# magenta/ddsp

Hardware: AMD Instinct MI355X
Metric: Msamples/s (Harmonic+FilteredNoise, 16kHz, 100 harmonics) (higher is better)
Workload: dtype f32 (Harmonic wavetables and the FilteredNoise FIR/IR products: 22-bit operands - fp16 hi/lo pairs on the MFMA matrix cores - with fp32 accumulation; everything else plain fp32, the frame phase prefix fp64)

## Files before the change

ddsp_amd/csrc/harmonic_table.hip:

```cpp
#include <hip/hip_runtime.h>
#include <hip/hip_ext.h>
#include <stdint.h>
#include <cstdlib>
#include <type_traits>
#include "../../include/ddsp_amd.h"
#include "common.h"
#include "split_f16.h"
#include "profile.h"
#include "harmonic_table.h"
#include "wavetable_coeffs.h"
#include "harm_table_frags.h"
#include "launch.h"
#include <mutex>

namespace ddsp {

static __device__ WtFragSet kWtFragSet6;
static __device__ WtFragSet kWtFragSet8;
static __device__ WtFragsWide kWtFragsWide;

constexpr int kWtT = 512;
constexpr int kWtHalf = kWtT / 2;
constexpr int kWtNQ = kWtT / 4;
template <int W> struct WtGeom {
  static constexpr int H = W <= 8 ? 4 : 8;
  static constexpr int TS = kWtHalf + 2 * H + 4;
};
constexpr int kWtRowTiles = 2;
constexpr int kWtRows = 16 * kWtRowTiles;
constexpr int kWtFrames = kWtRows - 1;
constexpr int kWtNT = 4;
template <int NK> struct WtPlane { static constexpr int PS = NK <= 2 ? 72 : 104; };

struct ChunkTables {
  double theta[kWtRows], w[kWtRows], dw[kWtRows];
  float f0[kWtRows + 2];
  int kA[kWtRows], kN[kWtRows];
  int cross;
  float4 cx[kWtRows];
  float ck[kWtRows];
};

template <int W> struct WtPoly;
template <> struct WtPoly<6> {
  static constexpr int DE = kWtDegE6, DO = kWtDegO6, K512 = 100;
  static constexpr float e(int p, int d) { return kWtE6[p * (DE + 1) + d]; }
  static constexpr float o(int p, int d) { return kWtO6[p * (DO + 1) + d]; }
};
template <> struct WtPoly<8> {
  static constexpr int DE = kWtDegE8, DO = kWtDegO8, K512 = 128;
  static constexpr float e(int p, int d) { return kWtE8[p * (DE + 1) + d]; }
  static constexpr float o(int p, int d) { return kWtO8[p * (DO + 1) + d]; }
};

template <> struct WtPoly<10> {
  static constexpr int DE = kWtDegE10, DO = kWtDegO10, K512 = 200;
  static constexpr float e(int p, int d) { return kWtE10[p * (DE + 1) + d]; }
  static constexpr float o(int p, int d) { return kWtO10[p * (DO + 1) + d]; }
};

constexpr int kWtWalker = 2;
constexpr int kWtSizer = 0;
constexpr unsigned kWtSlots = 0x73256104u;
struct WtDesc { int b, j0, nfr, fresh; };

struct WtSizeThresholds { float t64, t128, t256; };

struct TableArgs {
  int B, F, K, N, hop;
  int total_frames, frames_per_block;
  FastDiv f_div, tpf_div, seg_div;
  float nyquist, nyq_lo, nyq_hi;
  WtSizeThresholds size_thr;
  int amp_linear;
  int ragged;
  int rows16;
  double inv_sr, inv_2hop, hop_d, half_hm1;
};

struct WtWalk { int pos, pos_first, end, seg_left, base, rem, b, j; };

constexpr int kWtSegment = 2 * kWtFrames;

__device__ __forceinline__ WtDesc wt_next_chunk(WtWalk& w, const TableArgs& p) {
  WtDesc d{0, 0, 0, 0};
  if (w.pos >= w.end) return d;
  if (w.seg_left == 0) {
    uint32_t j;
    const int b = (int)fastdiv((uint32_t)w.pos, p.f_div, j);
    d.fresh = (w.pos == w.pos_first || (int)j == 0) ? 1 : 0;
    w.b = b;
    w.j = (int)j;
    uint32_t in_seg;
    (void)fastdiv(j, p.seg_div, in_seg);
    w.seg_left = min(min(w.end - w.pos, p.F - w.j), kWtSegment - (int)in_seg);
    const int n = (w.seg_left + kWtFrames - 1) / kWtFrames;
    w.base = w.seg_left / n;
    w.rem = w.seg_left - w.base * n;
  }
  const int len = w.base + (w.rem > 0 ? 1 : 0);
  if (w.rem > 0) --w.rem;
  d.b = w.b; d.j0 = w.j; d.nfr = len;
  w.pos += len; w.j += len; w.seg_left -= len;
  return d;
}

__device__ __forceinline__ int wt_table_size(float f0_min, const WtSizeThresholds& th) {
  return f0_min >= th.t64 ? 64 : f0_min >= th.t128 ? 128 : f0_min >= th.t256 ? 256 : kWtT;
}
inline WtSizeThresholds wt_size_thresholds(int K512, int K, float nyq_hi) {
  auto thr = [&](int T) -> float {
    const int kmax = K512 * T / 512;
    if (K <= kmax) return -__builtin_inff();
    return (float)((double)nyq_hi / (double)(kmax + 1) * (1.0 + 1e-6));
  };
  return WtSizeThresholds{thr(64), thr(128), thr(256)};
}

__device__ __forceinline__ WtDesc wt_read_desc(const WtDesc* ring, int slot) {
  const int4 v = *reinterpret_cast<const int4*>(ring + slot);
  WtDesc d;
  d.b = __builtin_amdgcn_readfirstlane(v.x);
  d.j0 = __builtin_amdgcn_readfirstlane(v.y);
  d.nfr = __builtin_amdgcn_readfirstlane(v.z);
  d.fresh = __builtin_amdgcn_readfirstlane(v.w);
  return d;
// ... 17 lines not shown
  __asm__("v_fma_mixhi_f16 %0, %1, %2, %3 op_sel:[1,0,0] op_sel_hi:[1,0,0]" : "+v"(r) : "v"(h), "v"(m), "v"(c2048[1]));
  return r;
#else
  return (h16x2){(__fp16)fmaf((float)h[0], -kLoScale, c2048[0]), (__fp16)fmaf((float)h[1], -kLoScale, c2048[1])};
#endif
}
__device__ __forceinline__ int wt_floor_int(float x) {
#if defined(__AMDGCN__)
  int r;
  __asm__("v_cvt_flr_i32_f32 %0, %1" : "=v"(r) : "v"(x));
  return r;
#else
  return (int)floorf(x);
#endif
}
__device__ __forceinline__ f32x2 wt_pk_fma_swap(f32x2 a, f32x2 b, f32x2 c) {
  return (f32x2){fmaf(a[0], b[1], c[0]), fmaf(a[1], b[0], c[1])};
}
__device__ __forceinline__ f32x2 wt_pk_plus(f32x2 o, f32x2 zz, f32x2 e) {
  return (f32x2){fmaf(o[0], zz[0], e[0]), fmaf(o[1], zz[0], e[1])};
}
__device__ __forceinline__ f32x2 wt_pk_minus(f32x2 o, f32x2 zz, f32x2 e) {
  return (f32x2){fmaf(-o[0], zz[0], e[0]), fmaf(-o[1], zz[0], e[1])};
}
template <int N>
__device__ __forceinline__ void wt_frags_landed(f32x4& a, f32x4& b, f32x4& c, f32x4& d) {
#if defined(__AMDGCN__)
  __asm__ volatile("s_waitcnt vmcnt(%4)" : "+v"(a), "+v"(b), "+v"(c), "+v"(d) : "n"(N));
#else
  (void)a; (void)b; (void)c; (void)d;
#endif
}
template <int N, class Fn>
__device__ __forceinline__ void wt_static_for(Fn&& f) {
  if constexpr (N > 0) {
    wt_static_for<N - 1>(f);
    f(std::integral_constant<int, N - 1>{});
  }
}
template <int W> struct WtPkCoefs {
  static constexpr int NG = W / 4, MID = (W / 2) & 1, DE = WtPoly<W>::DE, DO = WtPoly<W>::DO;
  f32x2 e[NG][DE + 1], o[NG][DO + 1], m[DE + 1];
  __device__ __forceinline__ void init() {
    wt_static_for<NG>([&](auto gg) {
      constexpr int g = decltype(gg)::value, pb = 2 * g + MID, pa = pb + 1;
      wt_static_for<DE + 1>([&](auto ss) {
// ... 66 lines not shown
    }
#pragma unroll
    for (int u = 0; u < NT; ++u) wp[u] = wt_pk_plus(oo[u], zz[u], ee[u]);
#pragma unroll
    for (int u = 0; u < NT; ++u) wm[u] = wt_pk_minus(oo[u], zz[u], ee[u]);
#pragma unroll
    for (int u = 0; u < NT; ++u) acc0[u] = wt_pk_fma(wp[u], lo0[u], acc0[u]);
#pragma unroll
    for (int u = 0; u < NT; ++u) acc1[u] = wt_pk_fma(wp[u], lo1[u], acc1[u]);
#pragma unroll
    for (int u = 0; u < NT; ++u) acc0[u] = wt_pk_fma_swap(wm[u], hi0[u], acc0[u]);
#pragma unroll
    for (int u = 0; u < NT; ++u) acc1[u] = wt_pk_fma_swap(wm[u], hi1[u], acc1[u]);
  });
}

typedef float* __restrict__ WtOutRestrict;
template <bool ADD> struct WtOut { typedef WtOutRestrict type; };
template <> struct WtOut<true> { typedef float* type; };

template <int W, int NK, bool ONE_TILE, bool ADD, bool ROWS16>
__global__ __launch_bounds__(1024) void harm_table_kernel(
    const float* __restrict__ amplitudes, const float* __restrict__ hd, const float* __restrict__ f0_all,
    typename WtOut<ADD>::type audio, float* __restrict__ ctl_amp, float* __restrict__ ctl_hd, const float* add_in, TableArgs p) {
  constexpr int kWtH = WtGeom<W>::H, kWtTS = WtGeom<W>::TS, kWtPS = WtPlane<NK>::PS;
  constexpr bool WIDE = NK > 2;
  __shared__ __attribute__((aligned(16))) float tab_all[2][kWtRows * kWtTS];
  __shared__ __attribute__((aligned(16))) _Float16 planes_all[3][4 * kWtRows * kWtPS];
  __shared__ ChunkTables t_all[2];
  __shared__ __attribute__((aligned(16))) WtDesc ring[8];
  __shared__ float amp_tab[3][kWtRows + 4];
  __shared__ int tsel[4];

  const int tid = threadIdx.x, lane = tid & 63;
  const int wave = __builtin_amdgcn_readfirstlane(tid >> 6);
  const bool is_t = wave < 4;
  const int F = p.F, K = p.K;
  const int K4 = (K + 3) >> 2;
  const float kLog10 = 2.302585092994046f;
  const int sub = lane >> 5, kq = lane & 31;
  const bool live = kq < K4;
  const float4* __restrict__ hd4 = reinterpret_cast<const float4*>(hd);
  const int mi = lane & 15, mg = lane >> 4;

  WtWalk walk;
  walk.pos = (int)blockIdx.x * p.frames_per_block;
  walk.pos_first = walk.pos;
  walk.end = min(walk.pos + p.frames_per_block, p.total_frames);
  walk.seg_left = 0; walk.base = 0; walk.rem = 0; walk.b = 0; walk.j = 0;
  if (wave == kWtWalker) {
    const WtDesc d0 = wt_next_chunk(walk, p), d1 = wt_next_chunk(walk, p);
    if (lane == 0) { ring[0] = d0; ring[1] = d1; }
  }
  __syncthreads();
  WtDesc dL{0, 0, 0, 0}, dA = wt_read_desc(ring, 0), dM{0, 0, 0, 0}, dB{0, 0, 0, 0};
  int pa = 0, pm = 2, pb = 1;

  int4 dnext = make_int4(0, 0, 0, 0);
  auto desc_issue = [&](int slot) { dnext = *reinterpret_cast<const int4*>(ring + slot); };
  auto desc_take = [&]() {
    dL.b = __builtin_amdgcn_readfirstlane(dnext.x);
    dL.j0 = __builtin_amdgcn_readfirstlane(dnext.y);
    dL.nfr = __builtin_amdgcn_readfirstlane(dnext.z);
    dL.fresh = __builtin_amdgcn_readfirstlane(dnext.w);
  };

  if (is_t) {
    const int rw = wave;
    f16x8 ahi[2][2][WIDE ? 1 : NK], alo[2][2][WIDE ? 1 : NK];
    int frag_T = 0;
    auto fetch_fragments = [&](int T) {
      const WtFragSet& set = W == 6 ? kWtFragSet6 : kWtFragSet8;
// ... 65 lines not shown
    auto fetch_segment = [&](const WtDesc& d, float& dst) {
      int lane_ = lane;
      DDSP_KEEP_IN_VGPR(lane_);
      uint32_t in_seg;
      (void)fastdiv((uint32_t)d.j0, p.seg_div, in_seg);
      load_issue(dst, f0_all + (size_t)d.b * F + min(d.j0 - (int)in_seg + lane_, F - 1));
    };
    auto fragments_landed = [&]() {
#if defined(__AMDGCN__)
      __asm__ volatile("s_waitcnt vmcnt(0)");
#pragma unroll
      for (int par = 0; par < 2; ++par)
#pragma unroll
        for (int tt = 0; tt < 2; ++tt)
#pragma unroll
          for (int ks = 0; ks < (WIDE ? 1 : NK); ++ks)
            __asm__ volatile("" : "+v"(ahi[par][tt][ks]), "+v"(alo[par][tt][ks]));
#endif
    };
    if constexpr (!WIDE) { fetch_fragments(kWtT); frag_T = kWtT; }
    int Tm = kWtT, Tm_ahead = kWtT;
    for (int tick = -2;; ++tick) {
      if (rw == 3 && dM.nfr > 0) {
        if (dM.fresh) before = row_prefix(dM);
        fetch_f0(dM);
      }
      WtDesc dN{0, 0, 0, 0};
      if (rw == 1 && dA.nfr > 0) fetch_amp(dA);
      if constexpr (!WIDE) {
        if (rw == kWtSizer) {
          dN = wt_read_desc(ring, (tick + 3) & 7);
          if (dN.nfr > 0) fetch_segment(dN, pseg);
          if (tick == -2 && dA.nfr > 0) fetch_segment(dA, pf_first);
        }
      }
      if constexpr (!WIDE) {
        Tm_ahead = tsel[(tick + 2) & 3];
        if (tick == -1) Tm = __builtin_amdgcn_readfirstlane(tsel[0]);
        if (dM.nfr > 0 && Tm != frag_T) {
          fetch_fragments(Tm);
          frag_T = Tm;
          fragments_landed();
        }
      }
      if (dM.nfr > 0 && !WIDE && Tm != kWtT) {
        if (rw < (Tm >> 6)) {
          const int half = Tm >> 1;
#pragma unroll
          for (int rt = 0; rt < kWtRowTiles; ++rt) {
            const _Float16* bsrc = planes_all[pm] + (16 * rt + mi) * kWtPS + 8 * mg;
            const float am = amp_tab[pm][16 * rt + mi], am_lo = am * (1.0f / kLoScale);
            f32x4 soe[2];
#pragma unroll
            for (int par = 0; par < 2; ++par) {
              const f16x8 bhi = *reinterpret_cast<const f16x8*>(bsrc + (0 * 2 + par) * kWtRows * kWtPS);
              const f16x8 blo = *reinterpret_cast<const f16x8*>(bsrc + (1 * 2 + par) * kWtRows * kWtPS);
              const f32x4 zero = {0.f, 0.f, 0.f, 0.f};
              const f32x4 acc = __builtin_amdgcn_mfma_f32_16x16x32_f16(ahi[par][0][0], bhi, zero, 0, 0, 0);
              f32x4 accx = __builtin_amdgcn_mfma_f32_16x16x32_f16(ahi[par][0][0], blo, zero, 0, 0, 0);
              accx = __builtin_amdgcn_mfma_f32_16x16x32_f16(alo[par][0][0], bhi, accx, 0, 0, 0);
              soe[par] = acc * am + accx * am_lo;
            }
            float* trow = tab_all[(tick + 1) & 1] + (16 * rt + mi) * kWtTS + kWtH;
            const int n0 = 16 * rw + 4 * mg;
            const f32x4 sp = soe[0] + soe[1], sm = soe[0] - soe[1];
            *reinterpret_cast<f32x4*>(trow + n0) = sp;
            *reinterpret_cast<f32x4*>(trow + (half - 4 - n0)) = (f32x4){sm.w, sm.z, sm.y, sm.x};
            if (n0 == 0) {
              *reinterpret_cast<f32x4*>(trow - 4) = (f32x4){-sp.w, -sp.z, -sp.y, -sp.x};
              *reinterpret_cast<f32x4*>(trow + half) = (f32x4){-sm.x, -sm.y, -sm.z, -sm.w};
            }
          }
        }
      } else if (dM.nfr > 0) {
#pragma unroll
       for (int rt = 0; rt < kWtRowTiles; ++rt) {
        const _Float16* bsrc = planes_all[pm] + (16 * rt + mi) * kWtPS + 8 * mg;
        f32x4 soe[2][2];
        const float am = amp_tab[pm][16 * rt + mi], am_lo = am * (1.0f / kLoScale);
#pragma unroll
        for (int par = 0; par < 2; ++par) {
          f32x4 acc[2], accx[2];
#pragma unroll
          for (int tt = 0; tt < 2; ++tt) {
            acc[tt] = (f32x4){0.f, 0.f, 0.f, 0.f};
            accx[tt] = (f32x4){0.f, 0.f, 0.f, 0.f};
          }
          if constexpr (WIDE) {
            f32x4 fr[NK][2][2];
            const char* fbase = reinterpret_cast<const char*>(kWtFragsWide.v) + 16384 * (rw * 2 + par);
            unsigned lane16 = 16u * (unsigned)lane;
            DDSP_KEEP_IN_VGPR(lane16);
            wt_static_for<NK>([&](auto kk) {
              constexpr int ks = decltype(kk)::value;
#pragma unroll
              for (int tt = 0; tt < 2; ++tt)
#pragma unroll
                for (int hl = 0; hl < 2; ++hl)
                  load_issue_spaced<1024 * ks>(fr[ks][tt][hl], fbase, lane16 + 4096u * (unsigned)(2 * tt + hl));
            });
            wt_static_for<NK>([&](auto kk) {
              constexpr int ks = decltype(kk)::value;
              const f16x8 bhi = *reinterpret_cast<const f16x8*>(bsrc + (0 * 2 + par) * kWtRows * kWtPS + wt_wide_kstep_base(ks));
              const f16x8 blo = *reinterpret_cast<const f16x8*>(bsrc + (1 * 2 + par) * kWtRows * kWtPS + wt_wide_kstep_base(ks));
              wt_frags_landed<4 * (NK - 1 - ks)>(fr[ks][0][0], fr[ks][0][1], fr[ks][1][0], fr[ks][1][1]);
#pragma unroll
              for (int tt = 0; tt < 2; ++tt)
                acc[tt] = __builtin_amdgcn_mfma_f32_16x16x32_f16(__builtin_bit_cast(f16x8, fr[ks][tt][0]), bhi, acc[tt], 0, 0, 0);
#pragma unroll
              for (int tt = 0; tt < 2; ++tt)
                accx[tt] = __builtin_amdgcn_mfma_f32_16x16x32_f16(__builtin_bit_cast(f16x8, fr[ks][tt][0]), blo, accx[tt], 0, 0, 0);
#pragma unroll
              for (int tt = 0; tt < 2; ++tt)
                accx[tt] = __builtin_amdgcn_mfma_f32_16x16x32_f16(__builtin_bit_cast(f16x8, fr[ks][tt][1]), bhi, accx[tt], 0, 0, 0);
            });
          } else {
#pragma unroll
          for (int ks = 0; ks < NK; ++ks) {
            const f16x8 bhi = *reinterpret_cast<const f16x8*>(bsrc + (0 * 2 + par) * kWtRows * kWtPS + 32 * ks);
            const f16x8 blo = *reinterpret_cast<const f16x8*>(bsrc + (1 * 2 + par) * kWtRows * kWtPS + 32 * ks);
#pragma unroll
            for (int tt = 0; tt < 2; ++tt)
              acc[tt] = __builtin_amdgcn_mfma_f32_16x16x32_f16(ahi[par][tt][ks], bhi, acc[tt], 0, 0, 0);
#pragma unroll
            for (int tt = 0; tt < 2; ++tt)
              accx[tt] = __builtin_amdgcn_mfma_f32_16x16x32_f16(ahi[par][tt][ks], blo, accx[tt], 0, 0, 0);
#pragma unroll
            for (int tt = 0; tt < 2; ++tt)
              accx[tt] = __builtin_amdgcn_mfma_f32_16x16x32_f16(alo[par][tt][ks], bhi, accx[tt], 0, 0, 0);
          }
          }
#pragma unroll
          for (int tt = 0; tt < 2; ++tt) soe[par][tt] = acc[tt] * am + accx[tt] * am_lo;
        }
        float* trow = tab_all[(tick + 1) & 1] + (16 * rt + mi) * kWtTS + kWtH;
#pragma unroll
        for (int tt = 0; tt < 2; ++tt) {
          const int n0 = 16 * (2 * rw + tt) + 4 * mg;
          const f32x4 so = soe[0][tt], se = soe[1][tt];
          const f32x4 sp = so + se;
          const f32x4 sm = so - se;
          *reinterpret_cast<f32x4*>(trow + n0) = sp;
          *reinterpret_cast<f32x4*>(trow + (kWtHalf - 4 - n0)) = (f32x4){sm.w, sm.z, sm.y, sm.x};
          if constexpr (kWtH == 4) {
          if (n0 == 0) {
            *reinterpret_cast<f32x4*>(trow - kWtH) = (f32x4){-sp.w, -sp.z, -sp.y, -sp.x};
            *reinterpret_cast<f32x4*>(trow + kWtHalf) = (f32x4){-sm.x, -sm.y, -sm.z, -sm.w};
          }
          } else {
          if (n0 < kWtH) {
            *reinterpret_cast<f32x4*>(trow - 4 - n0) = (f32x4){-sp.w, -sp.z, -sp.y, -sp.x};
            *reinterpret_cast<f32x4*>(trow + kWtHalf + n0) = (f32x4){-sm.x, -sm.y, -sm.z, -sm.w};
          }
          }
        }
       }
      }
      desc_issue((tick + 3) & 7);
// ... 20 lines not shown
          const unsigned hi15 = (unsigned)__builtin_amdgcn_readlane((int)(unsigned)((unsigned long long)bits15 >> 32), 15);
          const double first16 = __builtin_bit_cast(double, (long long)(((unsigned long long)hi15 << 32) | lo15));
          if (lane >= 16) incl += first16;
          const double s_excl = before + (incl - mine);
          const double run = p.hop_d * s_excl + (fa - (double)pf_first) * p.half_hm1;
          const double cyc = run * p.inv_sr;
          const float fmx = fmaxf(fj, fj1), fmn = fminf(fj, fj1);
          int kA = Kc, kN = Kc;
          if (fmx > 0.0f) kA = (int)fminf((float)Kc, floorf(p.nyq_lo * __builtin_amdgcn_rcpf(fmx)));
          if (fmn > 0.0f) kN = (int)fminf((float)Kc, floorf(p.nyq_hi * __builtin_amdgcn_rcpf(fmn)));
          kA = max(min(kA, kN), 0);
          const bool crossing = lane < nfr && kA < kN;
          const unsigned long long any = __builtin_amdgcn_ballot_w64(crossing);
          if (lane == 0) t.cross = any != 0ull ? 1 : 0;
          if (lane <= kWtRows) t.f0[lane] = fj;
          if (lane < kWtRows) {
            t.theta[lane] = cyc - floor(cyc);
            t.w[lane] = fa * p.inv_sr;
            t.dw[lane] = (fb - fa) * p.inv_sr * p.inv_2hop;
            t.kA[lane] = kA;
            t.kN[lane] = kN;
          }
          if (any != 0ull) {
            float4 cx = make_float4(0.0f, 0.0f, 0.0f, 0.0f);
            float ck = 0.0f;
            if (crossing) {
              const int k = kA;
              const float kfl = (float)(k + 1);
              const _Float16* pl = planes_all[pm] + ((k & 1) * kWtRows + lane) * kWtPS + (k >> 1);
              const float c0 = fmaf((float)pl[2 * kWtRows * kWtPS], 1.0f / kLoScale, (float)pl[0]);
              const float c1 = fmaf((float)pl[2 * kWtRows * kWtPS + kWtPS], 1.0f / kLoScale, (float)pl[kWtPS]);
              const float top = rn_mul(fj, kfl), bot = rn_mul(fj1, kfl);
              cx = make_float4(rn_mul(c0, amp_tab[pm][lane]), rn_mul(c1, amp_tab[pm][lane + 1]), top, rn_sub(bot, top));
              ck = kfl;
            }
            if (lane < kWtRows) { t.cx[lane] = cx; t.ck[lane] = ck; }
          }
          const long long bits31 = __builtin_bit_cast(long long, incl);
          const unsigned lo31 = (unsigned)__builtin_amdgcn_readlane((int)(unsigned)(bits31 & 0xffffffffll), 31);
          const unsigned hi31 = (unsigned)__builtin_amdgcn_readlane((int)(unsigned)((unsigned long long)bits31 >> 32), 31);
          before += __builtin_bit_cast(double, (long long)(((unsigned long long)hi31 << 32) | lo31));
        }
      }
      if (rw == 1 && dA.nfr > 0) {
        loads_landed(pamp);
        int lane_ = lane;
        DDSP_KEEP_IN_VGPR(lane_);
        const float a = exp_sigmoid_fast(pamp, kLog10, 2.0f, 1e-7f);
        if (lane_ <= kWtRows) amp_tab[pa][lane_] = a;
        if (ctl_amp != nullptr && lane_ < dA.nfr) ctl_amp[(size_t)dA.b * F + dA.j0 + lane_] = a;
      }
      if (rw == kWtSizer && (dN.nfr > 0 || (tick == -2 && dA.nfr > 0))) {
        loads_landed(pseg, pf_first);
        int lane_ = lane;
// ... 31 lines not shown
      const int hq = WIDE ? lane : kq;
      const bool live_h = WIDE ? lane < K4 : live;
      auto row_of = [&](int i, int pass) -> int { return 2 * u0 + NU * pass + i; };
      float kf[4], nyq_u[4];
#pragma unroll
      for (int u = 0; u < 4; ++u) {
        const bool alive = 4 * hq + u + 1 <= K;
        kf[u] = alive ? (float)(4 * hq + u + 1) : 0.0f;
        nyq_u[u] = alive ? p.nyquist : -1.0f;
      }
      struct Rows { f32x4 x[NU]; float f0[NU]; };
      Rows rows_a, rows_b;
      const unsigned kq16 = 16u * (unsigned)min(hq, K4 - 1), row_bytes = 4u * (unsigned)K;
      unsigned ku4[4];
#pragma unroll
      for (int u = 0; u < 4; ++u) ku4[u] = 4u * (unsigned)min(4 * hq + u, K - 1);
      auto prefetch = [&](const WtDesc& d, Rows& r, int pass) {
        const size_t r0 = (size_t)d.b * (size_t)F;
        const char* hb = reinterpret_cast<const char*>(hd) + r0 * row_bytes;
        const char* fb = reinterpret_cast<const char*>(f0_all) + r0 * 4;
        unsigned ro[NU];
#pragma unroll
        for (int i = 0; i < NU; ++i) {
          const unsigned jr = (unsigned)min(WIDE ? d.j0 + row_of(i, pass) : d.j0 + 2 * (u0 + i) + sub, F - 1);
          ro[i] = __umul24(jr, row_bytes);
          if constexpr (WIDE) load_issue_spaced<0>(r.f0[i], fb, 4u * jr);
          else load_issue(r.f0[i], fb, 4u * jr);
        }
        if constexpr (ROWS16) {
#pragma unroll
          for (int i = 0; i < NU; ++i) {
            if constexpr (WIDE) load_issue_spaced<0>(r.x[i], hb, ro[i] + kq16);
            else load_issue(r.x[i], hb, ro[i] + kq16);
          }
        } else {
#pragma unroll
          for (int i = 0; i < NU; ++i) {
            float e0, e1, e2, e3;
            if constexpr (WIDE) {
              load_issue_spaced<0>(e0, hb, ro[i] + ku4[0]);
              load_issue_spaced<0>(e1, hb, ro[i] + ku4[1]);
              load_issue_spaced<0>(e2, hb, ro[i] + ku4[2]);
              load_issue_spaced<0>(e3, hb, ro[i] + ku4[3]);
            } else {
            load_issue(e0, hb, ro[i] + ku4[0]);
            load_issue(e1, hb, ro[i] + ku4[1]);
            load_issue(e2, hb, ro[i] + ku4[2]);
// ... 8 lines not shown
        __asm__ volatile("s_waitcnt vmcnt(0)" : "+v"(r.x[0]), "+v"(r.x[1]), "+v"(r.x[2]), "+v"(r.x[3]), "+v"(r.f0[0]), "+v"(r.f0[1]),
                         "+v"(r.f0[2]), "+v"(r.f0[3]));
#else
        (void)r;
#endif
      };
      const f32x2 kf_o = {kf[0], kf[2]}, kf_e = {kf[1], kf[3]};
      auto exp_sigmoid2 = [&](f32x2 v) -> f32x2 {
        const f32x2 t = v * -1.4426950408889634f;
        const f32x2 e = (f32x2){__builtin_amdgcn_exp2f(t[0]), __builtin_amdgcn_exp2f(t[1])} + 1.0f;
        const f32x2 m = (f32x2){__builtin_amdgcn_logf(e[0]), __builtin_amdgcn_logf(e[1])} * -kLog10;
        const f32x2 g = {__builtin_amdgcn_exp2f(m[0]), __builtin_amdgcn_exp2f(m[1])};
        return __builtin_elementwise_fma(g, (f32x2){2.0f, 2.0f}, (f32x2){1e-7f, 1e-7f});
      };
      const float kHuge = 0x1p100f;
      const f32x2 nyq_o = {nyq_u[0] * kHuge, nyq_u[2] * kHuge}, nyq_e = {nyq_u[1] * kHuge, nyq_u[3] * kHuge};
      auto nyq_mask2 = [&](f32x2 e, float f0r, f32x2 kfp, f32x2 nyq_s) -> f32x2 {
        f32x2 prod;
        { _Pragma("clang fp contract(off)") prod = kfp * f0r; }
        const f32x2 y = __builtin_elementwise_fma(prod, (f32x2){-kHuge, -kHuge}, nyq_s);
        return (f32x2){__builtin_amdgcn_fmed3f(e[0], 0.0f, y[0]), __builtin_amdgcn_fmed3f(e[1], 0.0f, y[1])};
      };
      auto phase_a = [&](const WtDesc& d, _Float16* planes, const Rows& r, int pass) {
        const int nfr = d.nfr;
        f32x2 xo[NU], xe[NU];
        float part[NU], inv[NU];
#pragma unroll
        for (int i = 0; i < NU; ++i) {
          xo[i] = nyq_mask2(exp_sigmoid2((f32x2){r.x[i][0], r.x[i][2]}), r.f0[i], kf_o, nyq_o);
          xe[i] = nyq_mask2(exp_sigmoid2((f32x2){r.x[i][1], r.x[i][3]}), r.f0[i], kf_e, nyq_e);
        }
#pragma unroll
        for (int i = 0; i < NU; ++i) { const f32x2 h = xo[i] + xe[i]; part[i] = h[0] + h[1]; }
#pragma unroll
        for (int i = 0; i < NU; ++i) part[i] += dpp_mov0<0xB1, 0xF>(part[i]);
#pragma unroll
        for (int i = 0; i < NU; ++i) part[i] += dpp_mov0<0x4E, 0xF>(part[i]);
#pragma unroll
        for (int i = 0; i < NU; ++i) part[i] += dpp_mov0<0x141, 0xF>(part[i]);
#pragma unroll
        for (int i = 0; i < NU; ++i) part[i] += dpp_mov0<0x140, 0xF>(part[i]);
#pragma unroll
        for (int i = 0; i < NU; ++i) {
          part[i] = row_pair_sum(part[i]);
          if constexpr (WIDE) part[i] = wave_half_sum(part[i]);
          inv[i] = __builtin_amdgcn_rcpf(fmaxf(part[i], 1e-7f));
        }
        if (ctl_hd != nullptr) {
#pragma unroll
          for (int i = 0; i < NU; ++i) {
            const int arow = WIDE ? row_of(i, pass) : 2 * (u0 + i) + sub;
            const int crow = d.b * F + d.j0 + arow;
            if (arow < nfr) {
              const f32x2 ho = xo[i] * inv[i], he = xe[i] * inv[i];
              if constexpr (ROWS16) {
                if (live_h) reinterpret_cast<float4*>(ctl_hd)[(size_t)crow * K4 + hq] = make_float4(ho[0], he[0], ho[1], he[1]);
              } else {
                float* __restrict__ crow_p = ctl_hd + (size_t)crow * K + 4 * hq;
                const float h4[4] = {ho[0], he[0], ho[1], he[1]};
#pragma unroll
                for (int u = 0; u < 4; ++u)
                  if (4 * hq + u < K) crow_p[u] = h4[u];
              }
            }
          }
        }
#pragma unroll
        for (int i = 0; i < NU; ++i) {
          const f32x2 c[2] = {xo[i] * inv[i], xe[i] * inv[i]};
          _Float16* dst = planes + (WIDE ? row_of(i, pass) : 2 * (u0 + i) + sub) * kWtPS + 2 * hq;
#pragma unroll
          for (int par = 0; par < 2; ++par) {
            const h16x2 hi = __builtin_amdgcn_cvt_pkrtz(c[par][0], c[par][1]);
            const h16x2 lo = wt_rest_halves(c[par] * kLoScale, hi);
            if (!WIDE || 2 * hq < kWtPS) {
              *reinterpret_cast<h16x2*>(dst + (0 * 2 + par) * kWtRows * kWtPS) = hi;
              *reinterpret_cast<h16x2*>(dst + (1 * 2 + par) * kWtRows * kWtPS) = lo;
            }
          }
        }
      };
      prefetch(dA, rows_a, 0);
      if constexpr (WIDE) prefetch(dA, rows_b, 1);
      auto one_tick = [&](int tick, Rows& cur, Rows& next) -> bool {
        desc_issue((tick + 3) & 7);
        desc_take();
        rows_landed(cur);
        if constexpr (WIDE) {
          rows_landed(next);
          if (dA.nfr > 0) phase_a(dA, planes_all[pa], cur, 0);
          prefetch(dL, cur, 0);
          if (dA.nfr > 0) phase_a(dA, planes_all[pa], next, 1);
          prefetch(dL, next, 1);
        } else {
        prefetch(dL, next, 0);
        if (dA.nfr > 0) phase_a(dA, planes_all[pa], cur, 0);
        }
        __syncthreads();
        dB = dM; dM = dA; dA = dL;
        { const int t3 = pb; pb = pm; pm = pa; pa = t3; }
// ... 93 lines not shown
              out[u] = __builtin_bit_cast(float, __builtin_bit_cast(unsigned, v) ^ sgn[u]);
            }
            if (chunk_cross)
#pragma unroll
            for (int u = 0; u < NT; ++u) {
              const int kA = __builtin_amdgcn_readfirstlane(t.kA[q[u]]);
              const int kN = __builtin_amdgcn_readfirstlane(t.kN[q[u]]);
              if (kA < kN) {
                {
                  const float4 cx = t.cx[q[u]];
                  const float ck = t.ck[q[u]];
                  const float fk = rn_add(cx.z, rn_mul(cx.w, lerp[u]));
                  const float ak = fmaf(w_next[u], cx.y, rn_mul(w_cur[u], cx.x));
                  const float sv = sin_rev(fmaf(theta[u], ck, -rintf(theta[u] * ck)));
                  if (fk >= p.nyquist) out[u] = fmaf(-ak, sv, out[u]);
                }
                if (kA + 1 < kN) {
                  const float fj = t.f0[q[u]], fj1 = t.f0[q[u] + 1];
                  const float am0 = amp_tab[pb][q[u]], am1 = amp_tab[pb][q[u] + 1];
                  for (int k = kA + 1; k < kN; ++k) {
                    const float kfl = (float)(k + 1);
                    const float top = fj * kfl, bot = fj1 * kfl;
                    const float fk = rn_add(top, rn_mul(rn_sub(bot, top), lerp[u]));
                    const _Float16* pl = planes + ((k & 1) * kWtRows + q[u]) * kWtPS + (k >> 1);
                    const float c0 = fmaf((float)pl[2 * kWtRows * kWtPS], 1.0f / kLoScale, (float)pl[0]);
                    const float c1 = fmaf((float)pl[2 * kWtRows * kWtPS + kWtPS], 1.0f / kLoScale, (float)pl[kWtPS]);
                    const float ak = fmaf(w_next[u], rn_mul(c1, am1), rn_mul(w_cur[u], rn_mul(c0, am0)));
                    const float sv = sin_rev(fmaf(theta[u], kfl, -rintf(theta[u] * kfl)));
                    if (fk >= p.nyquist) out[u] = fmaf(-ak, sv, out[u]);
                  }
                }
              }
            }
            if (ADD)
#pragma unroll
              for (int u = 0; u < NT; ++u) out[u] += addv[u];
            if (!ragged) {
#pragma unroll
              for (int u = 0; u < NT; ++u) *reinterpret_cast<float*>(out_chunk + (o32 + 2048u * (unsigned)u)) = out[u];
            } else {
#pragma unroll
              for (int u = 0; u < NT; ++u)
                if (r[u] < hop) *reinterpret_cast<float*>(out_chunk + 4u * (unsigned)(q[u] * hop + r[u])) = out[u];
            }
          };
          for (int base = 0; base < n_tiles; base += kWtFrames) {
            const int left = min(n_tiles - base, kWtFrames);
            const int cnt = (left - slot + 7) >> 3;
            if (cnt >= 4) tiles(base + slot, std::integral_constant<int, 4>{});
            else if (cnt == 3) tiles(base + slot, std::integral_constant<int, 3>{});
            else if (cnt == 2) tiles(base + slot, std::integral_constant<int, 2>{});
            else if (cnt == 1) tiles(base + slot, std::integral_constant<int, 1>{});
          }
        }
        desc_take();
        if constexpr (!WIDE) Tf = (float)__builtin_amdgcn_readfirstlane(t_ahead);
        __syncthreads();
        dB = dM; dM = dA; dA = dL;
        { const int t3 = pb; pb = pm; pm = pa; pa = t3; }
        if (tick + 1 >= 0 && dB.nfr == 0) break;
      }
    }
  }
}

bool harm_table_ok(int F, int K, int N, const void* hd, const void* ctl_amp, const void* ctl_hd, unsigned flags,
                   int inputs_are_controls) {
  if (flags & DDSP_HARM_DIRECT_SUM) return false;
  if (!(flags & DDSP_HARM_SCALE_EXP_SIGMOID) || !(flags & DDSP_HARM_NORMALIZE_NYQUIST)) return false;
  if (inputs_are_controls || (ctl_amp == nullptr) != (ctl_hd == nullptr) || (flags >> 24) != 0) return false;
// ... 17 lines not shown
  if (W == 6) {
    if (!host6) { host6 = new WtFragSet; wt_fill_frag_set(host6, kWtInvPsi6_T512, (int)(sizeof(kWtInvPsi6_T512) / sizeof(float))); }
    rc = hipMemcpyToSymbol(HIP_SYMBOL(kWtFragSet6), host6, sizeof(WtFragSet));
  } else if (W == 8) {
    if (!host8) { host8 = new WtFragSet; wt_fill_frag_set(host8, kWtInvPsi8_T512, (int)(sizeof(kWtInvPsi8_T512) / sizeof(float))); }
    rc = hipMemcpyToSymbol(HIP_SYMBOL(kWtFragSet8), host8, sizeof(WtFragSet));
  } else {
    if (!host10) { host10 = new WtFragsWide; wt_fill_frags_wide(host10, kWtInvPsi10_T512, (int)(sizeof(kWtInvPsi10_T512) / sizeof(float))); }
    rc = hipMemcpyToSymbol(HIP_SYMBOL(kWtFragsWide), host10, sizeof(WtFragsWide));
  }
  if (rc != hipSuccess) return 1;
  done[dev][slot] = true;
  return 0;
}

int harm_table_prepare(int K) { return wt_upload_fragments(K <= 100 ? 6 : K <= 128 ? 8 : 10); }

int launch_harm_table(const float* amplitudes, const float* hd, const float* f0, float* audio, float* ctl_amp,
                     float* ctl_hd, const float* add_in, int B, int F, int K, int N, int sample_rate, unsigned flags,
                     hipStream_t st) {
  if ((long long)B * F >= (1ll << 31)) return DDSP_ERR_UNSUPPORTED;
  TableArgs p;
  p.B = B; p.F = F; p.K = K; p.N = N; p.hop = N / F;
  p.total_frames = B * F;
  p.f_div = make_fastdiv((uint32_t)F);
  p.tpf_div = make_fastdiv((uint32_t)((p.hop + 63) >> 6));
  p.ragged = (p.hop & 63) != 0 ? 1 : 0;
  p.seg_div = make_fastdiv((uint32_t)kWtSegment);
  if (wt_upload_fragments(K <= 100 ? 6 : K <= 128 ? 8 : 10) != 0) return DDSP_ERR_LAUNCH;
  p.nyquist = (float)(sample_rate / 2.0);
  p.nyq_lo = p.nyquist * (1.0f - 4e-6f);
  p.nyq_hi = p.nyquist * (1.0f + 4e-6f);
  p.size_thr = wt_size_thresholds(K <= 100 ? 100 : K <= 128 ? 128 : 200, K, p.nyq_hi);
  p.amp_linear = (flags & DDSP_HARM_AMP_LINEAR) ? 1 : 0;
  p.rows16 = ((K & 3) == 0 && (((uintptr_t)hd | (uintptr_t)ctl_hd) & 15) == 0) ? 1 : 0;
  p.inv_sr = 1.0 / (double)sample_rate;
  p.inv_2hop = 0.5 / (double)p.hop;
  p.hop_d = (double)p.hop;
  p.half_hm1 = ((double)p.hop - 1.0) * 0.5;
  static const int n_cu = [] {
    int dev = 0, v = 0;
    if (hipGetDevice(&dev) != hipSuccess ||
        hipDeviceGetAttribute(&v, hipDeviceAttributeMultiprocessorCount, dev) != hipSuccess || v <= 0)
      v = 256;
    return v;
  }();
  int blocks = (p.total_frames + kWtFrames - 1) / kWtFrames;
  if (blocks > n_cu) blocks = n_cu;
  p.frames_per_block = (p.total_frames + blocks - 1) / blocks;
  blocks = (p.total_frames + p.frames_per_block - 1) / p.frames_per_block;
  const dim3 grid((unsigned)blocks), block(1024);
  hipEvent_t ev0, ev1;
  profile_kernel_events(kHarmTable, &ev0, &ev1);
#define DDSP_LAUNCH_TABLE__(W, NK, ONE, ADD, R16)                                                                 \
  hipExtLaunchKernelGGL((harm_table_kernel<W, NK, ONE, ADD, R16>), grid, block, 0, st, ev0, ev1, 0, amplitudes, hd, f0, \
                        audio, ctl_amp, ctl_hd, add_in, p)
#define DDSP_LAUNCH_TABLE_(W, NK, ONE, ADD)                                                                     \
  do {                                                                                                         \
    if (p.rows16) DDSP_LAUNCH_TABLE__(W, NK, ONE, ADD, true);                                                  \
    else DDSP_LAUNCH_TABLE__(W, NK, ONE, ADD, false);                                                          \
  } while (0)
#define DDSP_LAUNCH_TABLE(W, NK)                                                                                \
  do {                                                                                                         \
    if (p.hop == 64) {                                                                                         \
      if (add_in != nullptr) DDSP_LAUNCH_TABLE_(W, NK, true, true);                                            \
      else DDSP_LAUNCH_TABLE_(W, NK, true, false);                                                             \
    } else {                                                                                                   \
      if (add_in != nullptr) DDSP_LAUNCH_TABLE_(W, NK, false, true);                                           \
      else DDSP_LAUNCH_TABLE_(W, NK, false, false);                                                            \
    }                                                                                                          \
  } while (0)
  if (K <= 64) DDSP_LAUNCH_TABLE(6, 1);
  else if (K <= 100) DDSP_LAUNCH_TABLE(6, 2);
  else if (K <= 128) DDSP_LAUNCH_TABLE(8, 2);
  else DDSP_LAUNCH_TABLE(10, 4);
#undef DDSP_LAUNCH_TABLE
#undef DDSP_LAUNCH_TABLE_
#undef DDSP_LAUNCH_TABLE__
  return check_launch();
// ... 4 lines not shown
```

Measured before the change: 120,500.

## Split frames into fixed 63-frame segments with row carry-over and host-planned block runs

The old chunker split each block's frame range into roughly even chunks that each recomputed their boundary row. Work now comes in fixed segments of a fresh 31-frame chunk followed by a 32-frame continuation chunk. The continuation reuses the previous chunk's last table row and coefficient planes by copying them in shared memory, so a boundary row is not rebuilt. A host-side planner, cached per (B, F, n_cu), assigns whole segments to blocks and passes per-block start indices as a kernel argument, which adds some LDS copies, extra shared rows and plan bookkeeping.

```diff
diff --git a/ddsp_amd/csrc/harm_table_plan.h b/ddsp_amd/csrc/harm_table_plan.h
--- /dev/null
+++ b/ddsp_amd/csrc/harm_table_plan.h
@@ -0,0 +1,71 @@
+#pragma once
+
+namespace ddsp {
+
+constexpr int kWtPlanFresh = 31;
+constexpr int kWtPlanCont = 32;
+constexpr int kWtPlanSegment = kWtPlanFresh + kWtPlanCont;
+constexpr int kWtPlanMaxBlocks = 320;
+
+struct WtPlan {
+  int segs_per_row;
+  int last_len;
+  int chunks_per_row;
+  long n_segs;
+  int blocks;
+  long chunks_max;
+  long first[kWtPlanMaxBlocks + 1];
+};
+
+inline int wt_plan_seg_chunks(int len) { return len > kWtPlanFresh ? 2 : 1; }
+
+inline long wt_plan_chunks_before(const WtPlan& p, long g) {
+  return (g / p.segs_per_row) * p.chunks_per_row + 2 * (g % p.segs_per_row);
+}
+inline long wt_plan_segs_within(const WtPlan& p, long x) {
+  const long g = (x / p.chunks_per_row) * p.segs_per_row + (x % p.chunks_per_row) / 2;
+  return g < p.n_segs ? g : p.n_segs;
+}
+
+inline long wt_plan_deal(WtPlan& p, long cap, int limit) {
+  long g = 0;
+  int i = 0;
+  while (g < p.n_segs) {
+    if (i == limit) return (long)limit + 1;
+    p.first[i++] = g;
+    g = wt_plan_segs_within(p, wt_plan_chunks_before(p, g) + cap);
+  }
+  p.first[i] = p.n_segs;
+  return i;
+}
+
+inline WtPlan plan_harm_table(int B, int F, int n_cu) {
+  WtPlan p{};
+  const int limit = n_cu < 1 ? 1 : n_cu < kWtPlanMaxBlocks ? n_cu : kWtPlanMaxBlocks;
+  p.segs_per_row = (F + kWtPlanSegment - 1) / kWtPlanSegment;
+  p.last_len = F - (p.segs_per_row - 1) * kWtPlanSegment;
+  p.chunks_per_row = 2 * (p.segs_per_row - 1) + wt_plan_seg_chunks(p.last_len);
+  p.n_segs = (long)B * p.segs_per_row;
+  const long total = (long)B * p.chunks_per_row;
+  long cap = (total + limit - 1) / limit;
+  const long largest = p.segs_per_row > 1 ? 2 : wt_plan_seg_chunks(p.last_len);
+  if (cap < largest) cap = largest;
+  while (wt_plan_deal(p, cap, limit) > limit) ++cap;
+  p.blocks = (int)wt_plan_deal(p, cap, limit);
+  p.chunks_max = 0;
+  for (int i = 0; i < p.blocks; ++i) {
+    const long c = wt_plan_chunks_before(p, p.first[i + 1]) - wt_plan_chunks_before(p, p.first[i]);
+    if (c > p.chunks_max) p.chunks_max = c;
+  }
+  return p;
+}
+
+struct WtPlanSeg { long row; int j0, len; };
+inline WtPlanSeg wt_plan_segment(const WtPlan& p, int F, long g) {
+  const long row = g / p.segs_per_row;
+  const int s = (int)(g % p.segs_per_row);
+  const int j0 = s * kWtPlanSegment;
+  return WtPlanSeg{row, j0, F - j0 < kWtPlanSegment ? F - j0 : kWtPlanSegment};
+}
+
+}
diff --git a/ddsp_amd/csrc/harmonic_table.hip b/ddsp_amd/csrc/harmonic_table.hip
--- a/ddsp_amd/csrc/harmonic_table.hip
+++ b/ddsp_amd/csrc/harmonic_table.hip
@@ -10,6 +10,7 @@
 #include "harmonic_table.h"
 #include "wavetable_coeffs.h"
 #include "harm_table_frags.h"
+#include "harm_table_plan.h"
 #include "launch.h"
 #include <mutex>
 
@@ -29,8 +30,12 @@
 constexpr int kWtRowTiles = 2;
 constexpr int kWtRows = 16 * kWtRowTiles;
 constexpr int kWtFrames = kWtRows - 1;
+constexpr int kWtTabRows = kWtRows + 1;
 constexpr int kWtNT = 4;
-template <int NK> struct WtPlane { static constexpr int PS = NK <= 2 ? 72 : 104; };
+template <int NK> struct WtPlane {
+  static constexpr int PS = NK <= 2 ? 72 : 104;
+  static constexpr int PL = (kWtTabRows * PS + 127) / 128 * 128;
+};
 
 struct ChunkTables {
   double theta[kWtRows], w[kWtRows], dw[kWtRows];
@@ -63,13 +68,16 @@
 constexpr int kWtSizer = 0;
 constexpr unsigned kWtSlots = 0x73256104u;
 struct WtDesc { int b, j0, nfr, fresh; };
+constexpr int kWtChunkPrefix = 1;
+constexpr int kWtChunkCont = 2;
+constexpr int kWtChunkFollowed = 4;
+__device__ __forceinline__ int wt_row_offset(const WtDesc& d) { return (d.fresh >> 1) & 1; }
 
 struct WtSizeThresholds { float t64, t128, t256; };
 
 struct TableArgs {
   int B, F, K, N, hop;
-  int total_frames, frames_per_block;
-  FastDiv f_div, tpf_div, seg_div;
+  FastDiv spr_div, tpf_div, seg_div;
   float nyquist, nyq_lo, nyq_hi;
   WtSizeThresholds size_thr;
   int amp_linear;
@@ -78,30 +86,30 @@
   double inv_sr, inv_2hop, hop_d, half_hm1;
 };
 
-struct WtWalk { int pos, pos_first, end, seg_left, base, rem, b, j; };
-
-constexpr int kWtSegment = 2 * kWtFrames;
+struct WtWalk { int seg, seg_first, seg_end, seg_left, b, j; };
+struct WtRuns { int first[kWtPlanMaxBlocks + 1]; };
+
+constexpr int kWtSegment = kWtFrames + kWtRows;
+static_assert(kWtSegment == kWtPlanSegment && kWtFrames == kWtPlanFresh && kWtRows == kWtPlanCont, "harm_table_plan.h");
+static_assert(kWtSegment + 1 <= 64, "the sizer reads a segment's f0 and the one behind with one load per lane");
 
 __device__ __forceinline__ WtDesc wt_next_chunk(WtWalk& w, const TableArgs& p) {
   WtDesc d{0, 0, 0, 0};
-  if (w.pos >= w.end) return d;
   if (w.seg_left == 0) {
-    uint32_t j;
-    const int b = (int)fastdiv((uint32_t)w.pos, p.f_div, j);
-    d.fresh = (w.pos == w.pos_first || (int)j == 0) ? 1 : 0;
-    w.b = b;
-    w.j = (int)j;
-    uint32_t in_seg;
-    (void)fastdiv(j, p.seg_div, in_seg);
-    w.seg_left = min(min(w.end - w.pos, p.F - w.j), kWtSegment - (int)in_seg);
-    const int n = (w.seg_left + kWtFrames - 1) / kWtFrames;
-    w.base = w.seg_left / n;
-    w.rem = w.seg_left - w.base * n;
+    if (w.seg >= w.seg_end) return d;
+    uint32_t s;
+    w.b = (int)fastdiv((uint32_t)w.seg, p.spr_div, s);
+    w.j = (int)s * kWtSegment;
+    w.seg_left = min(p.F - w.j, kWtSegment);
+    d.fresh = ((w.seg == w.seg_first || s == 0u) ? kWtChunkPrefix : 0) | (w.seg_left > kWtFrames ? kWtChunkFollowed : 0);
+    d.nfr = min(w.seg_left, kWtFrames);
+    ++w.seg;
+  } else {
+    d.fresh = kWtChunkCont;
+    d.nfr = w.seg_left;
   }
-  const int len = w.base + (w.rem > 0 ? 1 : 0);
-  if (w.rem > 0) --w.rem;
-  d.b = w.b; d.j0 = w.j; d.nfr = len;
-  w.pos += len; w.j += len; w.seg_left -= len;
+  d.b = w.b; d.j0 = w.j;
+  w.j += d.nfr; w.seg_left -= d.nfr;
   return d;
 }
 
@@ -165,6 +173,17 @@
 }
 __device__ __forceinline__ f32x2 wt_pk_minus(f32x2 o, f32x2 zz, f32x2 e) {
   return (f32x2){fmaf(-o[0], zz[0], e[0]), fmaf(-o[1], zz[0], e[1])};
+}
+template <bool FUSE_X>
+__device__ __forceinline__ f32x4 wt_scale_sums(f32x4 acc, float am, f32x4 accx, float am_lo) {
+  f32x4 prod;
+  if constexpr (FUSE_X) {
+    { _Pragma("clang fp contract(off)") prod = acc * am; }
+    return __builtin_elementwise_fma(accx, (f32x4){am_lo, am_lo, am_lo, am_lo}, prod);
+  } else {
+    { _Pragma("clang fp contract(off)") prod = accx * am_lo; }
+    return __builtin_elementwise_fma(acc, (f32x4){am, am, am, am}, prod);
+  }
 }
 template <int N>
 __device__ __forceinline__ void wt_frags_landed(f32x4& a, f32x4& b, f32x4& c, f32x4& d) {
@@ -277,11 +296,11 @@
 template <int W, int NK, bool ONE_TILE, bool ADD, bool ROWS16>
 __global__ __launch_bounds__(1024) void harm_table_kernel(
     const float* __restrict__ amplitudes, const float* __restrict__ hd, const float* __restrict__ f0_all,
-    typename WtOut<ADD>::type audio, float* __restrict__ ctl_amp, float* __restrict__ ctl_hd, const float* add_in, TableArgs p) {
-  constexpr int kWtH = WtGeom<W>::H, kWtTS = WtGeom<W>::TS, kWtPS = WtPlane<NK>::PS;
+    typename WtOut<ADD>::type audio, float* __restrict__ ctl_amp, float* __restrict__ ctl_hd, const float* add_in, TableArgs p, WtRuns runs) {
+  constexpr int kWtH = WtGeom<W>::H, kWtTS = WtGeom<W>::TS, kWtPS = WtPlane<NK>::PS, kWtPL = WtPlane<NK>::PL;
   constexpr bool WIDE = NK > 2;
-  __shared__ __attribute__((aligned(16))) float tab_all[2][kWtRows * kWtTS];
-  __shared__ __attribute__((aligned(16))) _Float16 planes_all[3][4 * kWtRows * kWtPS];
+  __shared__ __attribute__((aligned(16))) float tab_all[2][kWtTabRows * kWtTS];
+  __shared__ __attribute__((aligned(16))) _Float16 planes_all[3][4 * kWtPL];
   __shared__ ChunkTables t_all[2];
   __shared__ __attribute__((aligned(16))) WtDesc ring[8];
   __shared__ float amp_tab[3][kWtRows + 4];
@@ -299,10 +318,10 @@
   const int mi = lane & 15, mg = lane >> 4;
 
   WtWalk walk;
-  walk.pos = (int)blockIdx.x * p.frames_per_block;
-  walk.pos_first = walk.pos;
-  walk.end = min(walk.pos + p.frames_per_block, p.total_frames);
-  walk.seg_left = 0; walk.base = 0; walk.rem = 0; walk.b = 0; walk.j = 0;
+  walk.seg = runs.first[blockIdx.x];
+  walk.seg_first = walk.seg;
+  walk.seg_end = runs.first[blockIdx.x + 1];
+  walk.seg_left = 0; walk.b = 0; walk.j = 0;
   if (wave == kWtWalker) {
     const WtDesc d0 = wt_next_chunk(walk, p), d1 = wt_next_chunk(walk, p);
     if (lane == 0) { ring[0] = d0; ring[1] = d1; }
@@ -414,7 +433,7 @@
     int Tm = kWtT, Tm_ahead = kWtT;
     for (int tick = -2;; ++tick) {
       if (rw == 3 && dM.nfr > 0) {
-        if (dM.fresh) before = row_prefix(dM);
+        if (dM.fresh & kWtChunkPrefix) before = row_prefix(dM);
         fetch_f0(dM);
       }
       WtDesc dN{0, 0, 0, 0};
@@ -426,6 +445,16 @@
           if (tick == -2 && dA.nfr > 0) fetch_segment(dA, pf_first);
         }
       }
+      const int offM = wt_row_offset(dM);
+      if (rw == kWtSizer && dM.nfr > 0 && offM != 0) {
+        const f32x4* src = reinterpret_cast<const f32x4*>(tab_all[tick & 1] + kWtFrames * kWtTS);
+        f32x4* dst = reinterpret_cast<f32x4*>(tab_all[(tick + 1) & 1]);
+        static_assert(kWtTS % 4 == 0 && kWtTS / 4 <= 128, "a table row in two passes of 16-byte copies");
+        const f32x4 v0 = src[lane];
+        const f32x4 v1 = src[min(lane + 64, kWtTS / 4 - 1)];
+        dst[lane] = v0;
+        if (lane + 64 < kWtTS / 4) dst[lane + 64] = v1;
+      }
       if constexpr (!WIDE) {
         Tm_ahead = tsel[(tick + 2) & 3];
         if (tick == -1) Tm = __builtin_amdgcn_readfirstlane(tsel[0]);
@@ -440,20 +469,20 @@
           const int half = Tm >> 1;
 #pragma unroll
           for (int rt = 0; rt < kWtRowTiles; ++rt) {
-            const _Float16* bsrc = planes_all[pm] + (16 * rt + mi) * kWtPS + 8 * mg;
-            const float am = amp_tab[pm][16 * rt + mi], am_lo = am * (1.0f / kLoScale);
+            const _Float16* bsrc = planes_all[pm] + (offM + 16 * rt + mi) * kWtPS + 8 * mg;
+            const float am = amp_tab[pm][offM + 16 * rt + mi], am_lo = am * (1.0f / kLoScale);
             f32x4 soe[2];
 #pragma unroll
             for (int par = 0; par < 2; ++par) {
-              const f16x8 bhi = *reinterpret_cast<const f16x8*>(bsrc + (0 * 2 + par) * kWtRows * kWtPS);
-              const f16x8 blo = *reinterpret_cast<const f16x8*>(bsrc + (1 * 2 + par) * kWtRows * kWtPS);
+              const f16x8 bhi = *reinterpret_cast<const f16x8*>(bsrc + (0 * 2 + par) * kWtPL);
+              const f16x8 blo = *reinterpret_cast<const f16x8*>(bsrc + (1 * 2 + par) * kWtPL);
               const f32x4 zero = {0.f, 0.f, 0.f, 0.f};
               const f32x4 acc = __builtin_amdgcn_mfma_f32_16x16x32_f16(ahi[par][0][0], bhi, zero, 0, 0, 0);
               f32x4 accx = __builtin_amdgcn_mfma_f32_16x16x32_f16(ahi[par][0][0], blo, zero, 0, 0, 0);
               accx = __builtin_amdgcn_mfma_f32_16x16x32_f16(alo[par][0][0], bhi, accx, 0, 0, 0);
-              soe[par] = acc * am + accx * am_lo;
-            }
-            float* trow = tab_all[(tick + 1) & 1] + (16 * rt + mi) * kWtTS + kWtH;
+              soe[par] = wt_scale_sums<false>(acc, am, accx, am_lo);
+            }
+            float* trow = tab_all[(tick + 1) & 1] + (offM + 16 * rt + mi) * kWtTS + kWtH;
             const int n0 = 16 * rw + 4 * mg;
             const f32x4 sp = soe[0] + soe[1], sm = soe[0] - soe[1];
             *reinterpret_cast<f32x4*>(trow + n0) = sp;
@@ -467,9 +496,9 @@
       } else if (dM.nfr > 0) {
 #pragma unroll
        for (int rt = 0; rt < kWtRowTiles; ++rt) {
-        const _Float16* bsrc = planes_all[pm] + (16 * rt + mi) * kWtPS + 8 * mg;
+        const _Float16* bsrc = planes_all[pm] + (offM + 16 * rt + mi) * kWtPS + 8 * mg;
         f32x4 soe[2][2];
-        const float am = amp_tab[pm][16 * rt + mi], am_lo = am * (1.0f / kLoScale);
+        const float am = amp_tab[pm][offM + 16 * rt + mi], am_lo = am * (1.0f / kLoScale);
 #pragma unroll
         for (int par = 0; par < 2; ++par) {
           f32x4 acc[2], accx[2];
@@ -493,8 +522,8 @@
             });
             wt_static_for<NK>([&](auto kk) {
               constexpr int ks = decltype(kk)::value;
-              const f16x8 bhi = *reinterpret_cast<const f16x8*>(bsrc + (0 * 2 + par) * kWtRows * kWtPS + wt_wide_kstep_base(ks));
-              const f16x8 blo = *reinterpret_cast<const f16x8*>(bsrc + (1 * 2 + par) * kWtRows * kWtPS + wt_wide_kstep_base(ks));
+              const f16x8 bhi = *reinterpret_cast<const f16x8*>(bsrc + (0 * 2 + par) * kWtPL + wt_wide_kstep_base(ks));
+              const f16x8 blo = *reinterpret_cast<const f16x8*>(bsrc + (1 * 2 + par) * kWtPL + wt_wide_kstep_base(ks));
               wt_frags_landed<4 * (NK - 1 - ks)>(fr[ks][0][0], fr[ks][0][1], fr[ks][1][0], fr[ks][1][1]);
 #pragma unroll
               for (int tt = 0; tt < 2; ++tt)
@@ -509,8 +538,8 @@
           } else {
 #pragma unroll
           for (int ks = 0; ks < NK; ++ks) {
-            const f16x8 bhi = *reinterpret_cast<const f16x8*>(bsrc + (0 * 2 + par) * kWtRows * kWtPS + 32 * ks);
-            const f16x8 blo = *reinterpret_cast<const f16x8*>(bsrc + (1 * 2 + par) * kWtRows * kWtPS + 32 * ks);
+            const f16x8 bhi = *reinterpret_cast<const f16x8*>(bsrc + (0 * 2 + par) * kWtPL + 32 * ks);
+            const f16x8 blo = *reinterpret_cast<const f16x8*>(bsrc + (1 * 2 + par) * kWtPL + 32 * ks);
 #pragma unroll
             for (int tt = 0; tt < 2; ++tt)
               acc[tt] = __builtin_amdgcn_mfma_f32_16x16x32_f16(ahi[par][tt][ks], bhi, acc[tt], 0, 0, 0);
@@ -523,9 +552,9 @@
           }
           }
 #pragma unroll
-          for (int tt = 0; tt < 2; ++tt) soe[par][tt] = acc[tt] * am + accx[tt] * am_lo;
-        }
-        float* trow = tab_all[(tick + 1) & 1] + (16 * rt + mi) * kWtTS + kWtH;
+          for (int tt = 0; tt < 2; ++tt) soe[par][tt] = wt_scale_sums<!WIDE>(acc[tt], am, accx[tt], am_lo);
+        }
+        float* trow = tab_all[(tick + 1) & 1] + (offM + 16 * rt + mi) * kWtTS + kWtH;
 #pragma unroll
         for (int tt = 0; tt < 2; ++tt) {
           const int n0 = 16 * (2 * rw + tt) + 4 * mg;
@@ -592,14 +621,22 @@
             t.kN[lane] = kN;
           }
           if (any != 0ull) {
+            if (offM != 0 && lane < kWtPS / 2) {
+              const uint32_t* src = reinterpret_cast<const uint32_t*>(planes_all[pb] + kWtFrames * kWtPS) + lane;
+              uint32_t* dst = reinterpret_cast<uint32_t*>(planes_all[pm]) + lane;
+#pragma unroll
+              for (int pl4 = 0; pl4 < 4; ++pl4) dst[pl4 * (kWtPL / 2)] = src[pl4 * (kWtPL / 2)];
+            }
             float4 cx = make_float4(0.0f, 0.0f, 0.0f, 0.0f);
             float ck = 0.0f;
             if (crossing) {
               const int k = kA;
               const float kfl = (float)(k + 1);
-              const _Float16* pl = planes_all[pm] + ((k & 1) * kWtRows + lane) * kWtPS + (k >> 1);
-              const float c0 = fmaf((float)pl[2 * kWtRows * kWtPS], 1.0f / kLoScale, (float)pl[0]);
-              const float c1 = fmaf((float)pl[2 * kWtRows * kWtPS + kWtPS], 1.0f / kLoScale, (float)pl[kWtPS]);
+              const _Float16* pl = planes_all[pm] + (k & 1) * kWtPL + lane * kWtPS + (k >> 1);
+              const _Float16* pl_cur = (offM != 0 && lane == 0)
+                  ? planes_all[pb] + (k & 1) * kWtPL + kWtFrames * kWtPS + (k >> 1) : pl;
+              const float c0 = fmaf((float)pl_cur[2 * kWtPL], 1.0f / kLoScale, (float)pl_cur[0]);
+              const float c1 = fmaf((float)pl[2 * kWtPL + kWtPS], 1.0f / kLoScale, (float)pl[kWtPS]);
               const float top = rn_mul(fj, kfl), bot = rn_mul(fj1, kfl);
               cx = make_float4(rn_mul(c0, amp_tab[pm][lane]), rn_mul(c1, amp_tab[pm][lane + 1]), top, rn_sub(bot, top));
               ck = kfl;
@@ -677,7 +714,7 @@
         unsigned ro[NU];
 #pragma unroll
         for (int i = 0; i < NU; ++i) {
-          const unsigned jr = (unsigned)min(WIDE ? d.j0 + row_of(i, pass) : d.j0 + 2 * (u0 + i) + sub, F - 1);
+          const unsigned jr = (unsigned)min(d.j0 + wt_row_offset(d) + (WIDE ? row_of(i, pass) : 2 * (u0 + i) + sub), F - 1);
           ro[i] = __umul24(jr, row_bytes);
           if constexpr (WIDE) load_issue_spaced<0>(r.f0[i], fb, 4u * jr);
           else load_issue(r.f0[i], fb, 4u * jr);
@@ -732,7 +769,8 @@
         return (f32x2){__builtin_amdgcn_fmed3f(e[0], 0.0f, y[0]), __builtin_amdgcn_fmed3f(e[1], 0.0f, y[1])};
       };
       auto phase_a = [&](const WtDesc& d, _Float16* planes, const Rows& r, int pass) {
-        const int nfr = d.nfr;
+        const int off = wt_row_offset(d);
+        const int n_ctl = d.nfr + ((d.fresh & kWtChunkFollowed) ? 1 : 0);
         f32x2 xo[NU], xe[NU];
         float part[NU], inv[NU];
 #pragma unroll
@@ -759,9 +797,9 @@
         if (ctl_hd != nullptr) {
 #pragma unroll
           for (int i = 0; i < NU; ++i) {
-            const int arow = WIDE ? row_of(i, pass) : 2 * (u0 + i) + sub;
+            const int arow = off + (WIDE ? row_of(i, pass) : 2 * (u0 + i) + sub);
             const int crow = d.b * F + d.j0 + arow;
-            if (arow < nfr) {
+            if (arow < n_ctl) {
               const f32x2 ho = xo[i] * inv[i], he = xe[i] * inv[i];
               if constexpr (ROWS16) {
                 if (live_h) reinterpret_cast<float4*>(ctl_hd)[(size_t)crow * K4 + hq] = make_float4(ho[0], he[0], ho[1], he[1]);
@@ -778,14 +816,14 @@
 #pragma unroll
         for (int i = 0; i < NU; ++i) {
           const f32x2 c[2] = {xo[i] * inv[i], xe[i] * inv[i]};
-          _Float16* dst = planes + (WIDE ? row_of(i, pass) : 2 * (u0 + i) + sub) * kWtPS + 2 * hq;
+          _Float16* dst = planes + (off + (WIDE ? row_of(i, pass) : 2 * (u0 + i) + sub)) * kWtPS + 2 * hq;
 #pragma unroll
           for (int par = 0; par < 2; ++par) {
             const h16x2 hi = __builtin_amdgcn_cvt_pkrtz(c[par][0], c[par][1]);
             const h16x2 lo = wt_rest_halves(c[par] * kLoScale, hi);
             if (!WIDE || 2 * hq < kWtPS) {
-              *reinterpret_cast<h16x2*>(dst + (0 * 2 + par) * kWtRows * kWtPS) = hi;
-              *reinterpret_cast<h16x2*>(dst + (1 * 2 + par) * kWtRows * kWtPS) = lo;
+              *reinterpret_cast<h16x2*>(dst + (0 * 2 + par) * kWtPL) = hi;
+              *reinterpret_cast<h16x2*>(dst + (1 * 2 + par) * kWtPL) = lo;
             }
           }
         }
@@ -925,9 +963,9 @@
                     const float kfl = (float)(k + 1);
                     const float top = fj * kfl, bot = fj1 * kfl;
                     const float fk = rn_add(top, rn_mul(rn_sub(bot, top), lerp[u]));
-                    const _Float16* pl = planes + ((k & 1) * kWtRows + q[u]) * kWtPS + (k >> 1);
-                    const float c0 = fmaf((float)pl[2 * kWtRows * kWtPS], 1.0f / kLoScale, (float)pl[0]);
-                    const float c1 = fmaf((float)pl[2 * kWtRows * kWtPS + kWtPS], 1.0f / kLoScale, (float)pl[kWtPS]);
+                    const _Float16* pl = planes + (k & 1) * kWtPL + q[u] * kWtPS + (k >> 1);
+                    const float c0 = fmaf((float)pl[2 * kWtPL], 1.0f / kLoScale, (float)pl[0]);
+                    const float c1 = fmaf((float)pl[2 * kWtPL + kWtPS], 1.0f / kLoScale, (float)pl[kWtPS]);
                     const float ak = fmaf(w_next[u], rn_mul(c1, am1), rn_mul(w_cur[u], rn_mul(c0, am0)));
                     const float sv = sin_rev(fmaf(theta[u], kfl, -rintf(theta[u] * kfl)));
                     if (fk >= p.nyquist) out[u] = fmaf(-ak, sv, out[u]);
@@ -947,8 +985,8 @@
                 if (r[u] < hop) *reinterpret_cast<float*>(out_chunk + 4u * (unsigned)(q[u] * hop + r[u])) = out[u];
             }
           };
-          for (int base = 0; base < n_tiles; base += kWtFrames) {
-            const int left = min(n_tiles - base, kWtFrames);
+          for (int base = 0; base < n_tiles; base += kWtRows) {
+            const int left = min(n_tiles - base, kWtRows);
             const int cnt = (left - slot + 7) >> 3;
             if (cnt >= 4) tiles(base + slot, std::integral_constant<int, 4>{});
             else if (cnt == 3) tiles(base + slot, std::integral_constant<int, 3>{});
@@ -1012,8 +1050,6 @@
   if ((long long)B * F >= (1ll << 31)) return DDSP_ERR_UNSUPPORTED;
   TableArgs p;
   p.B = B; p.F = F; p.K = K; p.N = N; p.hop = N / F;
-  p.total_frames = B * F;
-  p.f_div = make_fastdiv((uint32_t)F);
   p.tpf_div = make_fastdiv((uint32_t)((p.hop + 63) >> 6));
   p.ragged = (p.hop & 63) != 0 ? 1 : 0;
   p.seg_div = make_fastdiv((uint32_t)kWtSegment);
@@ -1035,16 +1071,22 @@
       v = 256;
     return v;
   }();
-  int blocks = (p.total_frames + kWtFrames - 1) / kWtFrames;
-  if (blocks > n_cu) blocks = n_cu;
-  p.frames_per_block = (p.total_frames + blocks - 1) / blocks;
-  blocks = (p.total_frames + p.frames_per_block - 1) / p.frames_per_block;
-  const dim3 grid((unsigned)blocks), block(1024);
+  thread_local int plan_key[3] = {0, 0, 0};
+  thread_local WtRuns runs;
+  thread_local int plan_blocks = 0;
+  if (plan_key[0] != B || plan_key[1] != F || plan_key[2] != n_cu) {
+    const WtPlan plan = plan_harm_table(B, F, n_cu);
+    for (int i = 0; i <= plan.blocks; ++i) runs.first[i] = (int)plan.first[i];
+    plan_blocks = plan.blocks;
+    plan_key[0] = B; plan_key[1] = F; plan_key[2] = n_cu;
+  }
+  p.spr_div = make_fastdiv((uint32_t)((F + kWtSegment - 1) / kWtSegment));
+  const dim3 grid((unsigned)plan_blocks), block(1024);
   hipEvent_t ev0, ev1;
   profile_kernel_events(kHarmTable, &ev0, &ev1);
 #define DDSP_LAUNCH_TABLE__(W, NK, ONE, ADD, R16)                                                                 \
   hipExtLaunchKernelGGL((harm_table_kernel<W, NK, ONE, ADD, R16>), grid, block, 0, st, ev0, ev1, 0, amplitudes, hd, f0, \
-                        audio, ctl_amp, ctl_hd, add_in, p)
+                        audio, ctl_amp, ctl_hd, add_in, p, runs)
 #define DDSP_LAUNCH_TABLE_(W, NK, ONE, ADD)                                                                     \
   do {                                                                                                         \
     if (p.rows16) DDSP_LAUNCH_TABLE__(W, NK, ONE, ADD, true);                                                  \
```

New measurement: 120,900 (median of 6 runs). About the same (+0.3%).
